# Starlight0798/gymRL

Measured on AMD Instinct MI355X. Metric: env-steps/sec at N envs/GPU (PPO LunarLander), 1/2/4/8 GPUs + %HBM roofline, higher is better.
Workload: dtype f32; 1 GPU; PPO LunarLander-v3, 4096 vectorised envs per MI355X (BASELINE.json configs[1]); envs_per_gpu=4096, rollout_len=2048, num_epochs=10, num_minibatches=32, minibatch=262144, model=ActorCritic 8-256-256-{256-4,256-1} tanh, 200,965 params, parallelism=single GPU

## Files before the change

gymrl_amd/csrc/env_lunar_device.hpp:

```cpp
#pragma once
#include "env_common.hpp"

namespace gymrl {
namespace lunar {


constexpr float kScale = 30.0f;
constexpr float kW = 600.0f / kScale;
constexpr float kH = 400.0f / kScale;
constexpr float kHelipadY = kH / 4.0f;
constexpr float kLegDown = 18.0f / kScale;
constexpr float kLegAway = 20.0f / kScale;
constexpr float kDt = 1.0f / 50.0f;
constexpr int kVelIters = 180, kPosIters = 60, kMaxSteps = 1000;
constexpr float kLinearSlopSqMax = 0x1.a36e30p-16f;
constexpr float kLinearSlop = 0.005f, kAngularSlop = 2.0f / 180.0f * 3.14159265359f;
constexpr float kPolyRadius = 2.0f * kLinearSlop;
constexpr float kMaxLinCorr = 0.2f, kMaxAngCorr = 8.0f / 180.0f * 3.14159265359f;
constexpr float kBaumgarte = 0.2f;
constexpr float kMaxTranslation = 2.0f, kMaxRotation = 0.5f * 3.14159265359f;
constexpr float kTimeToSleep = 0.5f, kLinSleepTol = 0.01f, kAngSleepTol = 2.0f / 180.0f * 3.14159265359f;
constexpr float kMotorTorque = 40.0f;

__device__ constexpr float kInvM[3] = {0.20761245674740486f, 14.0625f, 14.0625f};
// ... 170 lines not shown
    i0x = v1x; i0y = v1y; i1x = v2x; i1y = v2y;
    id0 = 0u | ((uint32_t)pidx << 8) | (0u << 16) | (1u << 24);
    id1 = 0u | ((uint32_t)pidx << 8) | (0u << 16) | (1u << 24);
    ri1 = pidx; ri2 = pidx + 1 < NV ? pidx + 1 : 0;
    rv1x = wx[0]; rv1y = wy[0]; rv2x = wx[0]; rv2y = wy[0]; rnx = wnx[0]; rny = wny[0];
#pragma unroll
    for (int i = 0; i < NV; ++i) {
      if (i == ri1) { rv1x = wx[i]; rv1y = wy[i]; rnx = wnx[i]; rny = wny[i]; }
      if (i == ri2) { rv2x = wx[i]; rv2y = wy[i]; }
    }
  }
  const float sn1x = rny, sn1y = -rnx;
  const float so1 = dot2(sn1x, sn1y, rv1x, rv1y);
  const float so2 = dot2(-sn1x, -sn1y, rv2x, rv2y);

  float c0x, c0y, c1x, c1y; uint32_t cid0, cid1; int np = 0;
  {
    const float d0 = dot2(sn1x, sn1y, i0x, i0y) - so1;
    const float d1 = dot2(sn1x, sn1y, i1x, i1y) - so1;
    c0x = c0y = c1x = c1y = 0.0f; cid0 = cid1 = 0u;
    if (d0 <= 0.0f) { c0x = i0x; c0y = i0y; cid0 = id0; np = 1; }
    if (d1 <= 0.0f) { if (np == 0) { c0x = i1x; c0y = i1y; cid0 = id1; } else { c1x = i1x; c1y = i1y; cid1 = id1; } ++np; }
    if (d0 * d1 < 0.0f) {
      const float t = d0 / (d0 - d1);
      const float nxp = i0x + t * (i1x - i0x), nyp = i0y + t * (i1y - i0y);
      const uint32_t nid = (uint32_t)ri1 | (((id0 >> 8) & 0xFFu) << 8) | (0u << 16) | (1u << 24);
      if (np == 0) { c0x = nxp; c0y = nyp; cid0 = nid; } else { c1x = nxp; c1y = nyp; cid1 = nid; }
      ++np;
    }
  }
  if (np < 2) return;
  float e0x, e0y, e1x, e1y; uint32_t eid0, eid1; np = 0;
  {
    const float d0 = dot2(-sn1x, -sn1y, c0x, c0y) - so2;
    const float d1 = dot2(-sn1x, -sn1y, c1x, c1y) - so2;
    e0x = e0y = e1x = e1y = 0.0f; eid0 = eid1 = 0u;
    if (d0 <= 0.0f) { e0x = c0x; e0y = c0y; eid0 = cid0; np = 1; }
    if (d1 <= 0.0f) { if (np == 0) { e0x = c1x; e0y = c1y; eid0 = cid1; } else { e1x = c1x; e1y = c1y; eid1 = cid1; } ++np; }
    if (d0 * d1 < 0.0f) {
      const float t = d0 / (d0 - d1);
      const float nxp = c0x + t * (c1x - c0x), nyp = c0y + t * (c1y - c0y);
      const uint32_t nid = (uint32_t)ri2 | (((cid0 >> 8) & 0xFFu) << 8) | (0u << 16) | (1u << 24);
      if (np == 0) { e0x = nxp; e0y = nyp; eid0 = nid; } else { e1x = nxp; e1y = nyp; eid1 = nid; }
      ++np;
    }
  }
  if (np < 2) return;

  mf.faceB = use_edge ? 0 : 1;
  if (use_edge) { mf.lnx = rnx; mf.lny = rny; mf.lpx = rv1x; mf.lpy = rv1y; }
  else {
    mf.lnx = NX[0]; mf.lny = NY[0]; mf.lpx = VX[0]; mf.lpy = VY[0];
#pragma unroll
    for (int i = 0; i < NV; ++i) if (i == ri1) { mf.lnx = NX[i]; mf.lny = NY[i]; mf.lpx = VX[i]; mf.lpy = VY[i]; }
  }
  int cnt = 0;
#pragma unroll
  for (int k = 0; k < 2; ++k) {
    const float qx = k == 0 ? e0x : e1x, qy = k == 0 ? e0y : e1y;
    const uint32_t qid = k == 0 ? eid0 : eid1;
    const float sep = dot2(rnx, rny, qx - rv1x, qy - rv1y);
    if (sep <= radius) {
      float lx, ly; uint32_t key;
      if (use_edge) {
        const float dx = qx - px, dy = qy - py;
        lx = qc * dx + qs * dy; ly = -qs * dx + qc * dy;
        key = qid;
      } else {
        lx = qx; ly = qy;
        key = ((qid >> 8) & 0xFFu) | ((qid & 0xFFu) << 8) | (((qid >> 24) & 0xFFu) << 16) | (((qid >> 16) & 0xFFu) << 24);
      }
      if (cnt == 0) { mf.p[0].lpx = lx; mf.p[0].lpy = ly; mf.p[0].key = key; }
      else { mf.p[1].lpx = lx; mf.p[1].lpy = ly; mf.p[1].key = key; }
      ++cnt;
    }
  }
  mf.count = cnt;
}
__device__ __forceinline__ void body_xf(const Body& b, float lcy, float& px, float& py, float& qs, float& qc) {
  det_sincosf(b.a, &qs, &qc);
  px = b.cx - (qc * 0.0f - qs * lcy);
  py = b.cy - (qs * 0.0f + qc * lcy);
}

__device__ __forceinline__ float sel3(int mb, float a, float b, float c) { return mb == 0 ? a : (mb == 1 ? b : c); }
__device__ __forceinline__ Body select_body(const Body (&B)[3], int mb) {
  Body r;
  r.cx = sel3(mb, B[0].cx, B[1].cx, B[2].cx); r.cy = sel3(mb, B[0].cy, B[1].cy, B[2].cy);
  r.a = sel3(mb, B[0].a, B[1].a, B[2].a);
  r.vx = sel3(mb, B[0].vx, B[1].vx, B[2].vx); r.vy = sel3(mb, B[0].vy, B[1].vy, B[2].vy);
  r.w = sel3(mb, B[0].w, B[1].w, B[2].w);
  return r;
}

__device__ __forceinline__ void quad_share_velocity(Body (&B)[3], const Body& mine) {
  B[0].vx = quad_bcast<0>(mine.vx); B[0].vy = quad_bcast<0>(mine.vy); B[0].w = quad_bcast<0>(mine.w);
  B[1].vx = quad_bcast<1>(mine.vx); B[1].vy = quad_bcast<1>(mine.vy); B[1].w = quad_bcast<1>(mine.w);
  B[2].vx = quad_bcast<2>(mine.vx); B[2].vy = quad_bcast<2>(mine.vy); B[2].w = quad_bcast<2>(mine.w);
}
__device__ __forceinline__ void quad_share_position(Body (&B)[3], const Body& mine) {
  B[0].cx = quad_bcast<0>(mine.cx); B[0].cy = quad_bcast<0>(mine.cy); B[0].a = quad_bcast<0>(mine.a);
  B[1].cx = quad_bcast<1>(mine.cx); B[1].cy = quad_bcast<1>(mine.cy); B[1].a = quad_bcast<1>(mine.a);
  B[2].cx = quad_bcast<2>(mine.cx); B[2].cy = quad_bcast<2>(mine.cy); B[2].a = quad_bcast<2>(mine.a);
}

__device__ __forceinline__ void world_step(World& W, const Lds& lds, int role, int action, float disp0,
                                           float disp1, float fx, float fy, float& m_power, float& s_power) {
  Body(&B)[3] = W.b;
  const int mb = role == 3 ? 0 : role;
  const bool is_hull = mb == 0;
  const float mB_ = is_hull ? kInvM[0] : kInvM[1], iB_ = is_hull ? kInvI[0] : kInvI[1];
  const float lcy_ = is_hull ? kHullLcY : 0.0f;
  const float fr_ = is_hull ? sqrtf(0.1f * 0.1f) : sqrtf(0.2f * 0.1f);
  LUNAR_PROF_MARK(pt0);
  m_power = 0.0f; s_power = 0.0f;
  {
    float sn, cs;
    det_sincosf(B[0].a, &sn, &cs);
    const float tipx = sn, tipy = cs, sidex = -cs, sidey = sn;
    const float posx = B[0].cx - (cs * 0.0f - sn * kHullLcY);
    const float posy = B[0].cy - (sn * 0.0f + cs * kHullLcY);
    if (action == 2) {
      m_power = 1.0f;
      const float ox = tipx * (4.0f / kScale + 2.0f * disp0) + sidex * disp1;
      const float oy = -tipy * (4.0f / kScale + 2.0f * disp0) - sidey * disp1;
      const float ipx = posx + ox, ipy = posy + oy;
      const float Ix = -ox * 13.0f * m_power, Iy = -oy * 13.0f * m_power;
      B[0].vx += kInvM[0] * Ix; B[0].vy += kInvM[0] * Iy;
      B[0].w += kInvI[0] * cross2(ipx - B[0].cx, ipy - B[0].cy, Ix, Iy);
    }
    if (action == 1 || action == 3) {
      const float dir = (float)(action - 2);
      s_power = 1.0f;
      const float ox = tipx * disp0 + sidex * (3.0f * disp1 + dir * 12.0f / kScale);
      const float oy = -tipy * disp0 - sidey * (3.0f * disp1 + dir * 12.0f / kScale);
      const float ipx = posx + ox - tipx * 17.0f / kScale;
      const float ipy = posy + oy + tipy * 14.0f / kScale;
      const float Ix = -ox * 0.6f * s_power, Iy = -oy * 0.6f * s_power;
      B[0].vx += kInvM[0] * Ix; B[0].vy += kInvM[0] * Iy;
      B[0].w += kInvI[0] * cross2(ipx - B[0].cx, ipy - B[0].cy, Ix, Iy);
    }
  }

  uint32_t my_touch = 0u;
  bool my_contact = false;
  {
    const Body me = select_body(B, mb);
    float px, py, qs, qc;
    body_xf(me, lcy_, px, py, qs, qc);
    float minx = 3.4e38f, maxx = -3.4e38f, miny = 3.4e38f;
    if (is_hull) {
#pragma unroll
      for (int i = 0; i < 6; ++i) {
        const float x = (qc * kHullVx[i] - qs * kHullVy[i]) + px, y = (qs * kHullVx[i] + qc * kHullVy[i]) + py;
        minx = fminf(minx, x); maxx = fmaxf(maxx, x); miny = fminf(miny, y);
      }
    } else {
#pragma unroll
      for (int i = 0; i < 4; ++i) {
        const float x = (qc * kLegVx[i] - qs * kLegVy[i]) + px, y = (qs * kLegVx[i] + qc * kLegVy[i]) + py;
        minx = fminf(minx, x); maxx = fmaxf(maxx, x); miny = fminf(miny, y);
      }
    }
    int e_lo = (int)floorf((minx - 2.0f * kPolyRadius) * 0.5f);
    int e_hi = (int)floorf((maxx + 2.0f * kPolyRadius) * 0.5f);
    e_lo = e_lo < 0 ? 0 : e_lo;
// ... 241 lines not shown
    P2[L] = lane3(a23, a33, a13); Q2[L] = lane3(a13, a23, a33); A2[L] = lane3(a13, a11, a12);
    P3[L] = lane3(a23, a12, a22); Q3[L] = lane3(a12, a22, a23); A3[L] = lane3(a12, a13, a11);
    A3C[L] = lane3(a13, a23, 0.0f); D2[L] = lane3(a22, a11, 0.0f);
    MBv[L] = lane3(kInvM[L + 1], kInvM[L + 1], kInvI[L + 1]); IBz[L] = r2 ? kInvI[L + 1] : 0.0f;
  }
  const float MAv = lane3(kInvM[0], kInvM[0], kInvI[0]), IAz = r2 ? kInvI[0] : 0.0f;
  float VA = lane3(B[0].vx, B[0].vy, B[0].w);
  float VB[2] = {lane3(B[1].vx, B[1].vy, B[1].w), lane3(B[2].vx, B[2].vy, B[2].w)};
  float JI[2] = {lane3(W.j[0].ix, W.j[0].iy, W.j[0].iz), lane3(W.j[1].ix, W.j[1].iy, W.j[1].iz)};
  float IM[2] = {W.j[0].im, W.j[1].im};
  const float maxImp = h * kMotorTorque;
#define SB __builtin_amdgcn_sched_barrier(0)
#define USEL(c, a, b) (__builtin_unpredictable(c) ? (a) : (b))
  float zb[2];
  zb[1] = quad_perm<0xAA>(JI[1]) * A3C[1];
  zb[0] = 0.0f;
  float lim_nan[2] = {at_limit[0] ? lim_sign[0] : __builtin_nanf(""), at_limit[1] ? lim_sign[1] : __builtin_nanf("")};
  asm volatile("" : "+v"(lim_nan[0]), "+v"(lim_nan[1]));
  auto joints = [&]() {
#pragma unroll
    for (int jj = 0; jj < 2; ++jj) {
      const int L = 1 - jj;
      const bool lim = at_limit[L];
      float t = VB[L] - VA; SB;
      t = t - 0.3f * leg_sign(L); SB;
      float imp = -mmass[L] * t; SB;
      float nw = IM[L] + imp; SB;
      nw = __builtin_amdgcn_fmed3f(nw, -maxImp, maxImp); SB;
      imp = nw - IM[L]; IM[L] = nw; SB;
      const float mb_ = IBz[L] * imp; SB;
      VB[L] = VB[L] + mb_; SB;
      const float ma_ = IAz * imp; SB;
      VA = VA - ma_; SB;
      const float xb = quad_perm<0xAA>(VB[L]) * JPB[L]; SB;
      float c = VB[L] + xb; SB;
      const float xa = quad_perm<0xAA>(VA) * JPA[L]; SB;
      c = c - VA; SB;
      c = c - xa; SB;
      const float u1 = c * C1[L]; SB;
      const float zc = zb[L] - c; SB;
      const float q2 = quad_perm<kRot1>(c) * Q2[L]; SB;
      const float q3 = quad_perm<kRot2>(c) * Q3[L]; SB;
      const float m2 = c * P2[L] - q2; SB;
      const float m3 = c * P3[L] - q3; SB;
      float s1 = quad_perm<kRot1>(u1) + u1; SB;
      const float u2 = A2[L] * m2; SB;
      const float u3 = A3[L] * m3; SB;
      s1 = quad_perm<kRot2>(u1) + s1; SB;
      const float rr = USEL(lim, zc, -c); SB;
      float s2 = quad_perm<kRot1>(u2) + u2; SB;
      float s3 = quad_perm<kRot1>(u3) + u3; SB;
      const float d2r = D2[L] * rr; SB;
      s2 = quad_perm<kRot2>(u2) + s2; SB;
      s3 = quad_perm<kRot2>(u3) + s3; SB;
      const float r2_ = quad_perm<kSwap01>(rr) * K12[L]; SB;
      float sel = USEL(r1, s2, s3); SB;
      sel = USEL(r0, s1, sel); SB;
      const float nsol = -(det3i[L] * sel); SB;
      const float newJ = JI[L] + nsol; SB;
      const float uu = d2r - r2_; SB;
      const float u = det2i[L] * uu; SB;
      const float rt = quad_perm<0xAA>(newJ) * lim_nan[L]; SB;
      const float altz = USEL(lim, -JI[L], 0.0f); SB;
      const float alt = USEL(r2, altz, u); SB;
      float ip;
      asm("v_cmp_nge_f32 vcc, %1, 0\n\tv_cndmask_b32_e32 %0, %2, %3, vcc" : "=v"(ip) : "v"(rt), "v"(nsol), "v"(alt) : "vcc"); SB;
      JI[L] = JI[L] + ip; SB;
      zb[1 - L] = quad_perm<0xAA>(JI[1 - L]) * A3C[1 - L]; SB;
      const float ay = quad_perm<0x55>(ip) * jrAx[L]; SB;
      const float ax = quad_perm<0x00>(ip) * jrAy[L]; SB;
      const float by = quad_perm<0x55>(ip) * jrBx[L]; SB;
      const float bx = quad_perm<0x00>(ip) * jrBy[L]; SB;
      const float crA = ay - ax; SB;
      const float crB = by - bx; SB;
      const float wA = crA + ip; SB;
      const float wB = crB + ip; SB;
      float tA = USEL(r2, wA, ip); SB;
      float tB = USEL(r2, wB, ip); SB;
      tA = MAv * tA; SB;
      tB = MBv[L] * tB; SB;
      VA = VA - tA; SB;
      VB[L] = VB[L] + tB; SB;
    }
  };
#undef SB
#undef USEL
  auto contacts = [&]() {
    if (any_contact) {
      Body me;
      me.cx = me.cy = me.a = 0.0f;
      me.vx = sel3(mb, quad_bcast<0>(VA), quad_bcast<0>(VB[0]), quad_bcast<0>(VB[1]));
      me.vy = sel3(mb, quad_bcast<1>(VA), quad_bcast<1>(VB[0]), quad_bcast<1>(VB[1]));
      me.w = sel3(mb, quad_bcast<2>(VA), quad_bcast<2>(VB[0]), quad_bcast<2>(VB[1]));
#pragma unroll
      for (int s = 0; s < 2; ++s) {
        const int vcount = vcn[s];
        if (vcount > 0) {
          const float nx = vcf[s][VC_NX - 1], ny = vcf[s][VC_NY - 1], tx = ny, ty = -nx;
          const float rx0 = vcf[s][VC_RX0 - 1], ry0 = vcf[s][VC_RY0 - 1], rx1 = vcf[s][VC_RX1 - 1], ry1 = vcf[s][VC_RY1 - 1];
          float ni0 = vim[s][0], ti0 = vim[s][1], ni1 = vim[s][2], ti1 = vim[s][3];
          {
            const float dvx = me.vx + (-me.w * ry0), dvy = me.vy + (me.w * rx0);
            const float vt = dot2(dvx, dvy, tx, ty);
            float lam = vcf[s][VC_TM0 - 1] * (-vt);
            const float maxF = fr_ * ni0;
            const float nw = clampf(ti0 + lam, -maxF, maxF);
            lam = nw - ti0; ti0 = nw;
            const float Px = lam * tx, Py = lam * ty;
            me.vx += mB_ * Px; me.vy += mB_ * Py;
            me.w += iB_ * cross2(rx0, ry0, Px, Py);
          }
          if (vcount == 2) {
            const float dvx = me.vx + (-me.w * ry1), dvy = me.vy + (me.w * rx1);
            const float vt = dot2(dvx, dvy, tx, ty);
            float lam = vcf[s][VC_TM1 - 1] * (-vt);
            const float maxF = fr_ * ni1;
            const float nw = clampf(ti1 + lam, -maxF, maxF);
            lam = nw - ti1; ti1 = nw;
            const float Px = lam * tx, Py = lam * ty;
            me.vx += mB_ * Px; me.vy += mB_ * Py;
            me.w += iB_ * cross2(rx1, ry1, Px, Py);
          }
          if (vcount == 1) {
            const float dvx = me.vx + (-me.w * ry0), dvy = me.vy + (me.w * rx0);
            const float vn = dot2(dvx, dvy, nx, ny);
            float lam = -vcf[s][VC_NM0 - 1] * vn;
            const float nw = fmaxf(ni0 + lam, 0.0f);
            lam = nw - ni0; ni0 = nw;
            const float Px = lam * nx, Py = lam * ny;
            me.vx += mB_ * Px; me.vy += mB_ * Py;
            me.w += iB_ * cross2(rx0, ry0, Px, Py);
          } else {
            const float k11 = vcf[s][VC_K11 - 1], k12 = vcf[s][VC_K12 - 1], k22 = vcf[s][VC_K22 - 1];
            const float a1 = ni0, a2 = ni1;
            const float dv1x = me.vx + (-me.w * ry0), dv1y = me.vy + (me.w * rx0);
            const float dv2x = me.vx + (-me.w * ry1), dv2y = me.vy + (me.w * rx1);
            float vn1 = dot2(dv1x, dv1y, nx, ny), vn2 = dot2(dv2x, dv2y, nx, ny);
            const float b1 = vn1 - (k11 * a1 + k12 * a2);
            const float b2 = vn2 - (k12 * a1 + k22 * a2);
            float x1 = -(vcf[s][VC_I11 - 1] * b1 + vcf[s][VC_I12 - 1] * b2);
            float x2 = -(vcf[s][VC_I12 - 1] * b1 + vcf[s][VC_I22 - 1] * b2);
            bool ok = (x1 >= 0.0f && x2 >= 0.0f);
            if (!ok) {
              x1 = -vcf[s][VC_NM0 - 1] * b1; x2 = 0.0f;
              vn2 = k12 * x1 + b2;
              ok = (x1 >= 0.0f && vn2 >= 0.0f);
            }
            if (!ok) {
              x1 = 0.0f; x2 = -vcf[s][VC_NM1 - 1] * b2;
              vn1 = k12 * x2 + b1;
              ok = (x2 >= 0.0f && vn1 >= 0.0f);
            }
            if (!ok) {
              x1 = 0.0f; x2 = 0.0f;
              ok = (b1 >= 0.0f && b2 >= 0.0f);
            }
            if (ok) {
              const float d1 = x1 - a1, d2 = x2 - a2;
              const float P1x = d1 * nx, P1y = d1 * ny, P2x = d2 * nx, P2y = d2 * ny;
              me.vx += mB_ * (P1x + P2x); me.vy += mB_ * (P1y + P2y);
              me.w += iB_ * (cross2(rx0, ry0, P1x, P1y) + cross2(rx1, ry1, P2x, P2y));
              ni0 = x1; ni1 = x2;
            }
          }
          vim[s][0] = ni0; vim[s][1] = ti0;
          if (vcount == 2) { vim[s][2] = ni1; vim[s][3] = ti1; }
        }
      }
      VA = lane3(quad_bcast<0>(me.vx), quad_bcast<0>(me.vy), quad_bcast<0>(me.w));
      VB[0] = lane3(quad_bcast<1>(me.vx), quad_bcast<1>(me.vy), quad_bcast<1>(me.w));
      VB[1] = lane3(quad_bcast<2>(me.vx), quad_bcast<2>(me.vy), quad_bcast<2>(me.w));
    }
  };
  if (__builtin_amdgcn_ballot_w64(any_contact) == 0ull) {
#pragma nounroll
    for (int it = 0; it < kVelIters; ++it) joints();
  } else {
#pragma nounroll
    for (int it = 0; it < kVelIters; ++it) { joints(); contacts(); }
  }
  B[0].vx = quad_bcast<0>(VA); B[0].vy = quad_bcast<1>(VA); B[0].w = quad_bcast<2>(VA);
#pragma unroll
  for (int L = 0; L < 2; ++L) {
    B[L + 1].vx = quad_bcast<0>(VB[L]); B[L + 1].vy = quad_bcast<1>(VB[L]); B[L + 1].w = quad_bcast<2>(VB[L]);
    W.j[L].ix = quad_bcast<0>(JI[L]); W.j[L].iy = quad_bcast<1>(JI[L]); W.j[L].iz = quad_bcast<2>(JI[L]);
    W.j[L].im = quad_bcast<2>(IM[L]);
  }
  LUNAR_PROF_MARK(pt3);
  LUNAR_PROF_ADD(lds, 2, pt2, pt3);
#ifdef GYMRL_LUNAR_PROF
  const bool wave_contact = __builtin_amdgcn_ballot_w64(any_contact) != 0ull;
  LUNAR_PROF_ADD(lds, wave_contact ? 6 : 7, pt2, pt3);
#endif
  if (my_contact) {
#pragma unroll
    for (int s = 0; s < 2; ++s) {
      if (vcn[s] > 0) {
        lds.mf(s, MF_P0 + P_NI) = vim[s][0]; lds.mf(s, MF_P0 + P_TI) = vim[s][1];
        if (vcn[s] == 2) { lds.mf(s, MF_P1 + P_NI) = vim[s][2]; lds.mf(s, MF_P1 + P_TI) = vim[s][3]; }
      }
    }
  }

#pragma unroll
  for (int b = 0; b < 3; ++b) {
    float tx = h * B[b].vx, ty = h * B[b].vy;
    if (dot2(tx, ty, tx, ty) > kMaxTranslation * kMaxTranslation) {
      const float ratio = kMaxTranslation / sqrtf(dot2(tx, ty, tx, ty));
      B[b].vx *= ratio; B[b].vy *= ratio;
    }
    const float rot = h * B[b].w;
    if (rot * rot > kMaxRotation * kMaxRotation) {
      const float ratio = kMaxRotation / fabsf(rot);
      B[b].w *= ratio;
    }
    B[b].cx += h * B[b].vx; B[b].cy += h * B[b].vy; B[b].a += h * B[b].w;
  }

  LUNAR_PROF_MARK(pt4);
  LUNAR_PROF_ADD(lds, 3, pt3, pt4);
#ifdef GYMRL_LUNAR_PROF
  int prof_pos_iters = 0;
#endif
  bool position_solved = false;
  float plim_value[2], plim_slop[2], plim_lo[2], plim_hi[2];
#pragma unroll
  for (int L = 0; L < 2; ++L) {
    const bool lower = W.j[L].state == 1;
    plim_value[L] = lower ? joint_lower(L) : joint_upper(L);
    plim_slop[L] = lower ? kAngularSlop : -kAngularSlop;
    plim_lo[L] = lower ? -kMaxAngCorr : 0.0f;
    plim_hi[L] = lower ? 0.0f : kMaxAngCorr;
  }
  int pcnt[2] = {0, 0};
  bool pfaceB[2] = {false, false};
  float plnx[2], plny[2], plpx[2], plpy[2], pqx[2][2], pqy[2][2];
#pragma unroll
  for (int s = 0; s < 2; ++s) {
    plnx[s] = plny[s] = plpx[s] = plpy[s] = 0.0f;
    pqx[s][0] = pqx[s][1] = pqy[s][0] = pqy[s][1] = 0.0f;
    if (my_contact) {
      pcnt[s] = (int)lds.mu(s, MF_COUNT);
      pfaceB[s] = lds.mu(s, MF_FACEB) != 0u;
      plnx[s] = lds.mf(s, MF_LNX); plny[s] = lds.mf(s, MF_LNY);
      plpx[s] = lds.mf(s, MF_LPX); plpy[s] = lds.mf(s, MF_LPY);
#pragma unroll
      for (int k = 0; k < 2; ++k) {
        pqx[s][k] = lds.mf(s, MF_P0 + 5 * k + P_LPX); pqy[s][k] = lds.mf(s, MF_P0 + 5 * k + P_LPY);
      }
    }
  }
#pragma nounroll
  for (int it = 0; it < kPosIters; ++it) {
    float min_sep = 0.0f;
    if (any_contact) {
      Body me = select_body(B, mb);
      float my_min = 0.0f;
#pragma unroll
      for (int s = 0; s < 2; ++s) {
        const int cnt = pcnt[s];
        if (cnt > 0) {
          const bool faceB = pfaceB[s];
          const float lnx = plnx[s], lny = plny[s], lpx = plpx[s], lpy = plpy[s];
#pragma unroll
          for (int k = 0; k < 2; ++k) {
            if (k < cnt) {
              const float qx = pqx[s][k], qy = pqy[s][k];
              float px, py, qs, qc;
              body_xf(me, lcy_, px, py, qs, qc);
              float nx, ny, ptx, pty, sep;
              if (!faceB) {
                nx = lnx; ny = lny;
                const float clx = (qc * qx - qs * qy) + px, cly = (qs * qx + qc * qy) + py;
                sep = dot2(clx - lpx, cly - lpy, nx, ny) - kPolyRadius - kPolyRadius;
                ptx = clx; pty = cly;
// ... 414 lines not shown
```

gymrl_amd/csrc/rollout_lunar.hip:

```cpp
#include "env_lunar_device.hpp"
#include "mlp_device.hpp"
#include "policy_device.hpp"
#include "mhc_policy_device.hpp"

using namespace gymrl;
using namespace gymrl::lunar;
namespace M = gymrl::mlp;

namespace {

constexpr int kThreads = M::kWaves * 64;
constexpr int kActions = 4, kObs = 8;
constexpr int kGaeChunk = 16;
constexpr int kDynFloats = M::kBufs * M::kRows * M::kStride + M::kRows * M::kInStride + M::kRows * M::kHeadStride;
constexpr int kDynBytes = 96 * 1024;
constexpr int kDynBytesMhc = 32 * 1024;
static_assert(kDynFloats * 4 <= kDynBytes, "LDS carve-up");

__global__ __launch_bounds__(kThreads) void rollout_lunar_kernel(gymrl_rollout_lunar_args a, gymrl_mlp_desc d) {
  extern __shared__ __attribute__((aligned(16))) float dyn_lds[];
  __shared__ uint32_t lds_words[kLdsWords * kEnvBlock];
  __shared__ uint32_t lds_words_refill[kLdsWords * kEnvBlock];
  __shared__ uint32_t lds_park[kParkWords * kEnvBlock];
  float (*lds)[M::kRows * M::kStride] = reinterpret_cast<float (*)[M::kRows * M::kStride]>(dyn_lds);
  float* xin = dyn_lds + M::kBufs * M::kRows * M::kStride;
  float* head = xin + M::kRows * M::kInStride;
  const int tid = threadIdx.x, wave = tid >> 6, lane = tid & 63;
  const int N = a.n_envs, T = a.T;
  const int m0 = blockIdx.x * M::kRows;
  const int t_end = a.t0 + a.nsteps;
  const int role = lane & 3, row = lane >> 2, i = m0 + row;
  const bool valid = i < N;
  const LunarState st(a.env_state, N);
#ifdef GYMRL_LUNAR_PROF
  constexpr int kProfSlots = 24;
  unsigned long long* const wprof = a.wg_ticks ? reinterpret_cast<unsigned long long*>(a.wg_ticks) + 2 * gridDim.x + kProfSlots * blockIdx.x : nullptr;
  Lds slds_{lds_words + lane, wprof, lds_park + lane};
  if (a.wg_ticks && valid) { slds_.envp = reinterpret_cast<unsigned long long*>(a.wg_ticks) + (2 + kProfSlots) * gridDim.x + i; slds_.envn = N; }
  const Lds slds = slds_;
  if (wprof && lane == 0) {
    wprof[20 + wave] = (unsigned long long)__builtin_amdgcn_s_getreg(4 | (31 << 11)) |
                       ((unsigned long long)__builtin_amdgcn_s_getreg(20 | (31 << 11)) << 32);
  }
#else
  const Lds slds{lds_words + lane, lds_park + lane};
#endif
#ifdef GYMRL_LUNAR_PROF
  const Lds rlds{lds_words_refill + lane, nullptr};
#else
  const Lds rlds{lds_words_refill + lane};
#endif
  const double gl = (double)(float)(a.gamma * a.lam);
  if (a.wg_ticks && tid == 0) a.wg_ticks[2 * blockIdx.x] = wall_clock64();

  for (int e = tid; e < M::kRows * M::kInStride; e += kThreads) xin[e] = 0.0f;
  __syncthreads();
  for (int e = tid; e < M::kRows * kObs; e += kThreads) {
    const int r = e / kObs, c = e - r * kObs;
    if (m0 + r < N) xin[r * M::kInStride + c] = a.obs[((size_t)a.t0 * N + m0 + r) * kObs + c];
  }
  const uint32_t vdefer = M::deferrable_stages(d, kActions);
  for (int t = a.t0; t <= t_end; ++t) {
    const bool tail = t == t_end;
    if (tail && t_end != T) break;
    LUNAR_PROF_MARK(rtb);
    __syncthreads();
    LUNAR_PROF_MARK(rt0);
    if (wave == 0) LUNAR_PROF_ADD(slds, 16, rtb, rt0);
    M::forward_tile(d, lds, xin, head, m0, N, tid, vdefer);
    LUNAR_PROF_MARK(rt1);
    if (wave == 0) LUNAR_PROF_ADD(slds, 8, rt0, rt1);
    auto value_part = [&]() {
      const float v = head[row * M::kHeadStride + kActions];
      if (valid && role == 0) {
        if (a.gae_running && t > 0) {
          const int tp = t - 1;
          const size_t o = (size_t)tp * N + i;
          double2* agg = reinterpret_cast<double2*>(a.gae_workspace) + (size_t)(tp / kGaeChunk) * N;
          gae_online_compose(a.rew[o], a.done[o], a.val[o], v, a.gamma, gl, (tp % kGaeChunk) == 0,
                             (tp % kGaeChunk) == kGaeChunk - 1 || tp == T - 1, a.gae_running, agg, N, i);
        }
        if (tail) {
          a.next_value[i] = v;
          if (a.gae_carry && a.gae_running) {
            const int C = (T + kGaeChunk - 1) / kGaeChunk;
            const double2* agg0 = reinterpret_cast<const double2*>(a.gae_workspace);
            static_assert(sizeof(lds_words_refill) >= sizeof(double2) * kGaeCarrySeg * kEnvBlock / 4, "carry scratch");
            gae_carry_scan(agg0, C, N, i, reinterpret_cast<double*>(const_cast<double2*>(agg0) + (size_t)C * N),
                           reinterpret_cast<double2*>(lds_words_refill) + row, kEnvBlock / 4);
          }
        } else a.val[(size_t)t * N + i] = v;
      }
    };
    if (wave == 2 && vdefer) {
      M::forward_deferred(d, lds, head, m0, N, lane, vdefer);
      value_part();
#ifdef GYMRL_LUNAR_PROF
      if (wprof && lane == 0) wprof[17] += wall_clock64() - rt1;
#endif
    }
    const bool refill_wave = wave == 1;
    if (wave == 0 || (refill_wave && !tail && a.refill)) {
      int act = 0;
      if (!refill_wave) {
        float z[kActions];
#pragma unroll
        for (int k = 0; k < kActions; ++k) z[k] = head[row * M::kHeadStride + k];
        if (!vdefer) value_part();
        if (!tail) {
          float lp, H;
          const size_t o = (size_t)t * N + (valid ? i : 0);
          act = categorical_pick<kActions>(z, a.noise_exp ? a.noise_exp + o * kActions : nullptr, a.seed,
                                           (uint64_t)(a.env_id0 + i), a.counter0 + (uint64_t)t, 0, lp, H);
          if (valid && role == 0) { a.act[o] = act; a.logp[o] = lp; }
        }
      }
      if (!tail) {
        const StepOut out{a.obs + (size_t)(t + 1) * N * kObs, nullptr, a.rew + (size_t)t * N, nullptr, nullptr,
// ... 190 lines not shown
```

Measured before the change: 7.092 million env-steps/s.

## Add specialized resting-contact velocity solver path for single-point leg contacts

Adds a specialized velocity-iteration path for waves where every contacting lane is a leg with exactly one contact point. It replaces the general contacts() lambda with a compact one-point friction+normal solve done directly on quad-distributed velocities, skipping the broadcast and reassembly of the general path. It also adds profiling counters and enlarges the profile slot count under the profiling macro. The risk is a numerical mismatch against the general solver, plus extra register pressure from the precomputed resting-contact values.

```diff
diff --git a/gymrl_amd/csrc/env_lunar_device.hpp b/gymrl_amd/csrc/env_lunar_device.hpp
--- a/gymrl_amd/csrc/env_lunar_device.hpp
+++ b/gymrl_amd/csrc/env_lunar_device.hpp
@@ -683,6 +683,83 @@
       VA = VA - tA; SB;
       VB[L] = VB[L] + tB; SB;
     }
+  };
+  const bool rs_slot1 = vcn[0] == 0;
+  auto rs_vc = [&](int f) { return rs_slot1 ? vcf[1][f - 1] : vcf[0][f - 1]; };
+  const float rs_nx = rs_vc(VC_NX), rs_ny = rs_vc(VC_NY), rs_tx = rs_ny, rs_ty = -rs_nx;
+  const float rs_rx = rs_vc(VC_RX0), rs_ry = rs_vc(VC_RY0), rs_tm = rs_vc(VC_TM0), rs_nm = rs_vc(VC_NM0);
+  const float rs_mB = kInvM[1], rs_iB = kInvI[1], rs_fr = sqrtf(0.2f * 0.1f);
+  float rs_ni = rs_slot1 ? vim[1][0] : vim[0][0], rs_ti = rs_slot1 ? vim[1][1] : vim[0][1];
+  const bool rs_has0 = quad_bcast_u<1>(my_contact ? 1u : 0u) != 0u, rs_has1 = quad_bcast_u<2>(my_contact ? 1u : 0u) != 0u;
+  const bool rs_0x = rs_has0 && r0, rs_0y = rs_has0 && r1, rs_0w = rs_has0 && r2;
+  const bool rs_1x = rs_has1 && r0, rs_1y = rs_has1 && r1, rs_1w = rs_has1 && r2;
+  auto resting = [&]() {
+    const float in_x1 = quad_bcast<0>(VB[1]); SB;
+    const float in_y1 = quad_bcast<1>(VB[1]); SB;
+    const float in_w0 = quad_bcast<2>(VB[0]); SB;
+    const float in_x0 = quad_bcast<0>(VB[0]); SB;
+    float vy = USEL(r1, VB[0], in_y1); SB;
+    float w = USEL(r2, VB[1], in_w0); SB;
+    float vx = USEL(r1, in_x0, in_x1); SB;
+    {
+      const float wy = -w * rs_ry; SB;
+      const float wx = w * rs_rx; SB;
+      const float dvx = vx + wy; SB;
+      const float dvy = vy + wx; SB;
+      const float p1 = dvx * rs_tx; SB;
+      const float p2 = dvy * rs_ty; SB;
+      const float vt = p1 + p2; SB;
+      float lam = rs_tm * (-vt); SB;
+      const float maxF = rs_fr * rs_ni; SB;
+      const float su = rs_ti + lam; SB;
+      const float nw = clampf(su, -maxF, maxF); SB;
+      lam = nw - rs_ti; rs_ti = nw; SB;
+      const float Px = lam * rs_tx; SB;
+      const float Py = lam * rs_ty; SB;
+      const float ax = rs_mB * Px; SB;
+      const float ay = rs_mB * Py; SB;
+      vx = vx + ax; SB;
+      vy = vy + ay; SB;
+      const float c1 = rs_rx * Py; SB;
+      const float c2 = rs_ry * Px; SB;
+      const float cr = c1 - c2; SB;
+      const float aw = rs_iB * cr; SB;
+      w = w + aw; SB;
+    }
+    {
+      const float wy = -w * rs_ry; SB;
+      const float wx = w * rs_rx; SB;
+      const float dvx = vx + wy; SB;
+      const float dvy = vy + wx; SB;
+      const float p1 = dvx * rs_nx; SB;
+      const float p2 = dvy * rs_ny; SB;
+      const float vn = p1 + p2; SB;
+      float lam = -rs_nm * vn; SB;
+      const float su = rs_ni + lam; SB;
+      const float nw = fmaxf(su, 0.0f); SB;
+      lam = nw - rs_ni; rs_ni = nw; SB;
+      const float Px = lam * rs_nx; SB;
+      const float Py = lam * rs_ny; SB;
+      const float ax = rs_mB * Px; SB;
+      const float ay = rs_mB * Py; SB;
+      vx = vx + ax; SB;
+      vy = vy + ay; SB;
+      const float c1 = rs_rx * Py; SB;
+      const float c2 = rs_ry * Px; SB;
+      const float cr = c1 - c2; SB;
+      const float aw = rs_iB * cr; SB;
+      w = w + aw; SB;
+    }
+    const float out_x0 = quad_bcast<1>(vx); SB;
+    const float out_x1 = quad_bcast<2>(vx); SB;
+    const float out_y1 = quad_bcast<2>(vy); SB;
+    const float out_w0 = quad_bcast<1>(w); SB;
+    VB[0] = USEL(rs_0y, vy, VB[0]); SB;
+    VB[1] = USEL(rs_1w, w, VB[1]); SB;
+    VB[0] = USEL(rs_0x, out_x0, VB[0]); SB;
+    VB[1] = USEL(rs_1x, out_x1, VB[1]); SB;
+    VB[1] = USEL(rs_1y, out_y1, VB[1]); SB;
+    VB[0] = USEL(rs_0w, out_w0, VB[0]); SB;
   };
 #undef SB
 #undef USEL
@@ -773,9 +850,15 @@
       VB[1] = lane3(quad_bcast<2>(me.vx), quad_bcast<2>(me.vy), quad_bcast<2>(me.w));
     }
   };
+  const bool lane_general = my_contact && (is_hull || vcn[0] + vcn[1] != 1);
+  const bool wave_resting = __builtin_amdgcn_ballot_w64(my_contact) != 0ull && __builtin_amdgcn_ballot_w64(lane_general) == 0ull;
   if (__builtin_amdgcn_ballot_w64(any_contact) == 0ull) {
 #pragma nounroll
     for (int it = 0; it < kVelIters; ++it) joints();
+  } else if (wave_resting) {
+#pragma nounroll
+    for (int it = 0; it < kVelIters; ++it) { joints(); resting(); }
+    if (rs_slot1) { vim[1][0] = rs_ni; vim[1][1] = rs_ti; } else { vim[0][0] = rs_ni; vim[0][1] = rs_ti; }
   } else {
 #pragma nounroll
     for (int it = 0; it < kVelIters; ++it) { joints(); contacts(); }
@@ -792,6 +875,21 @@
 #ifdef GYMRL_LUNAR_PROF
   const bool wave_contact = __builtin_amdgcn_ballot_w64(any_contact) != 0ull;
   LUNAR_PROF_ADD(lds, wave_contact ? 6 : 7, pt2, pt3);
+  if (lds.prof && (threadIdx.x & 63) == 0) {
+    lds.prof[24] += wave_resting ? 1ull : 0ull; lds.prof[25] += (wave_contact && !wave_resting) ? 1ull : 0ull;
+    lds.prof[26] += wave_resting ? pt3 - pt2 : 0ull;
+  }
+  {
+    const bool one_mf = my_contact && !is_hull && (vcn[0] == 0 || vcn[1] == 0);
+    const bool one_pt = one_mf && vcn[0] + vcn[1] == 1, two_pt = one_mf && vcn[0] + vcn[1] == 2;
+    const unsigned long long mc = __builtin_amdgcn_ballot_w64(my_contact && role != 3), m1 = __builtin_amdgcn_ballot_w64(one_mf),
+                             mp = __builtin_amdgcn_ballot_w64(one_pt), m2 = __builtin_amdgcn_ballot_w64(two_pt);
+    if (lds.prof && (threadIdx.x & 63) == 0) {
+      lds.prof[27] += (mc != 0ull && m2 == mc) ? 1ull : 0ull; lds.prof[28] += (mc != 0ull && m1 == mc && mp != mc && m2 != mc) ? 1ull : 0ull;
+      lds.prof[29] += (unsigned long long)__builtin_popcountll(mc); lds.prof[30] += (unsigned long long)__builtin_popcountll(mp);
+      lds.prof[31] += (unsigned long long)__builtin_popcountll(m2);
+    }
+  }
 #endif
   if (my_contact) {
 #pragma unroll
diff --git a/gymrl_amd/csrc/rollout_lunar.hip b/gymrl_amd/csrc/rollout_lunar.hip
--- a/gymrl_amd/csrc/rollout_lunar.hip
+++ b/gymrl_amd/csrc/rollout_lunar.hip
@@ -33,7 +33,7 @@
   const bool valid = i < N;
   const LunarState st(a.env_state, N);
 #ifdef GYMRL_LUNAR_PROF
-  constexpr int kProfSlots = 24;
+  constexpr int kProfSlots = 32;
   unsigned long long* const wprof = a.wg_ticks ? reinterpret_cast<unsigned long long*>(a.wg_ticks) + 2 * gridDim.x + kProfSlots * blockIdx.x : nullptr;
   Lds slds_{lds_words + lane, wprof, lds_park + lane};
   if (a.wg_ticks && valid) { slds_.envp = reinterpret_cast<unsigned long long*>(a.wg_ticks) + (2 + kProfSlots) * gridDim.x + i; slds_.envn = N; }
```

New measurement: 7.278 million env-steps/s, median of 6. 1.03x the previous value.

## Specialize contact solver per wave contact pattern with branchless selects

Applied to the files above, without the earlier changes.

The velocity-iteration contact solver becomes a template specialised on slot count, one- versus two-point manifolds and hull contact. Wave-wide ballots pick the cheapest variant for the whole 180-iteration loop. Inside each variant the data-dependent branches (point count, the block-solver LCP cases) are replaced by computing every candidate and choosing with unpredictable selects, which removes divergence. The cost is redundant arithmetic per lane and more code size and register pressure, and the reordered block-solver cases could subtly change results if the selection logic is wrong.

```diff
diff --git a/gymrl_amd/csrc/env_lunar_device.hpp b/gymrl_amd/csrc/env_lunar_device.hpp
--- a/gymrl_amd/csrc/env_lunar_device.hpp
+++ b/gymrl_amd/csrc/env_lunar_device.hpp
@@ -276,6 +276,8 @@
   px = b.cx - (qc * 0.0f - qs * lcy);
   py = b.cy - (qs * 0.0f + qc * lcy);
 }
+
+template <int V> struct IntC { static constexpr int value = V; };
 
 __device__ __forceinline__ float sel3(int mb, float a, float b, float c) { return mb == 0 ? a : (mb == 1 ? b : c); }
 __device__ __forceinline__ Body select_body(const Body (&B)[3], int mb) {
@@ -686,99 +688,124 @@
   };
 #undef SB
 #undef USEL
-  auto contacts = [&]() {
-    if (any_contact) {
-      Body me;
-      me.cx = me.cy = me.a = 0.0f;
-      me.vx = sel3(mb, quad_bcast<0>(VA), quad_bcast<0>(VB[0]), quad_bcast<0>(VB[1]));
-      me.vy = sel3(mb, quad_bcast<1>(VA), quad_bcast<1>(VB[0]), quad_bcast<1>(VB[1]));
-      me.w = sel3(mb, quad_bcast<2>(VA), quad_bcast<2>(VB[0]), quad_bcast<2>(VB[1]));
-#pragma unroll
-      for (int s = 0; s < 2; ++s) {
-        const int vcount = vcn[s];
-        if (vcount > 0) {
-          const float nx = vcf[s][VC_NX - 1], ny = vcf[s][VC_NY - 1], tx = ny, ty = -nx;
-          const float rx0 = vcf[s][VC_RX0 - 1], ry0 = vcf[s][VC_RY0 - 1], rx1 = vcf[s][VC_RX1 - 1], ry1 = vcf[s][VC_RY1 - 1];
-          float ni0 = vim[s][0], ti0 = vim[s][1], ni1 = vim[s][2], ti1 = vim[s][3];
-          {
-            const float dvx = me.vx + (-me.w * ry0), dvy = me.vy + (me.w * rx0);
-            const float vt = dot2(dvx, dvy, tx, ty);
-            float lam = vcf[s][VC_TM0 - 1] * (-vt);
-            const float maxF = fr_ * ni0;
-            const float nw = clampf(ti0 + lam, -maxF, maxF);
-            lam = nw - ti0; ti0 = nw;
-            const float Px = lam * tx, Py = lam * ty;
-            me.vx += mB_ * Px; me.vy += mB_ * Py;
-            me.w += iB_ * cross2(rx0, ry0, Px, Py);
-          }
-          if (vcount == 2) {
-            const float dvx = me.vx + (-me.w * ry1), dvy = me.vy + (me.w * rx1);
-            const float vt = dot2(dvx, dvy, tx, ty);
-            float lam = vcf[s][VC_TM1 - 1] * (-vt);
-            const float maxF = fr_ * ni1;
-            const float nw = clampf(ti1 + lam, -maxF, maxF);
-            lam = nw - ti1; ti1 = nw;
-            const float Px = lam * tx, Py = lam * ty;
-            me.vx += mB_ * Px; me.vy += mB_ * Py;
-            me.w += iB_ * cross2(rx1, ry1, Px, Py);
-          }
-          if (vcount == 1) {
-            const float dvx = me.vx + (-me.w * ry0), dvy = me.vy + (me.w * rx0);
-            const float vn = dot2(dvx, dvy, nx, ny);
-            float lam = -vcf[s][VC_NM0 - 1] * vn;
-            const float nw = fmaxf(ni0 + lam, 0.0f);
-            lam = nw - ni0; ni0 = nw;
-            const float Px = lam * nx, Py = lam * ny;
-            me.vx += mB_ * Px; me.vy += mB_ * Py;
-            me.w += iB_ * cross2(rx0, ry0, Px, Py);
-          } else {
-            const float k11 = vcf[s][VC_K11 - 1], k12 = vcf[s][VC_K12 - 1], k22 = vcf[s][VC_K22 - 1];
-            const float a1 = ni0, a2 = ni1;
-            const float dv1x = me.vx + (-me.w * ry0), dv1y = me.vy + (me.w * rx0);
-            const float dv2x = me.vx + (-me.w * ry1), dv2y = me.vy + (me.w * rx1);
-            float vn1 = dot2(dv1x, dv1y, nx, ny), vn2 = dot2(dv2x, dv2y, nx, ny);
-            const float b1 = vn1 - (k11 * a1 + k12 * a2);
-            const float b2 = vn2 - (k12 * a1 + k22 * a2);
-            float x1 = -(vcf[s][VC_I11 - 1] * b1 + vcf[s][VC_I12 - 1] * b2);
-            float x2 = -(vcf[s][VC_I12 - 1] * b1 + vcf[s][VC_I22 - 1] * b2);
-            bool ok = (x1 >= 0.0f && x2 >= 0.0f);
-            if (!ok) {
-              x1 = -vcf[s][VC_NM0 - 1] * b1; x2 = 0.0f;
-              vn2 = k12 * x1 + b2;
-              ok = (x1 >= 0.0f && vn2 >= 0.0f);
-            }
-            if (!ok) {
-              x1 = 0.0f; x2 = -vcf[s][VC_NM1 - 1] * b2;
-              vn1 = k12 * x2 + b1;
-              ok = (x2 >= 0.0f && vn1 >= 0.0f);
-            }
-            if (!ok) {
-              x1 = 0.0f; x2 = 0.0f;
-              ok = (b1 >= 0.0f && b2 >= 0.0f);
-            }
-            if (ok) {
-              const float d1 = x1 - a1, d2 = x2 - a2;
-              const float P1x = d1 * nx, P1y = d1 * ny, P2x = d2 * nx, P2y = d2 * ny;
-              me.vx += mB_ * (P1x + P2x); me.vy += mB_ * (P1y + P2y);
-              me.w += iB_ * (cross2(rx0, ry0, P1x, P1y) + cross2(rx1, ry1, P2x, P2y));
-              ni0 = x1; ni1 = x2;
-            }
-          }
-          vim[s][0] = ni0; vim[s][1] = ti0;
-          if (vcount == 2) { vim[s][2] = ni1; vim[s][3] = ti1; }
+  bool c_use[2], c_two[2], c_one[2];
+#pragma unroll
+  for (int s = 0; s < 2; ++s) { c_use[s] = vcn[s] > 0; c_two[s] = vcn[s] == 2; c_one[s] = vcn[s] == 1; }
+#define USEL(c, a, b) (__builtin_unpredictable(c) ? (a) : (b))
+  auto contacts = [&](auto slots_c, auto one_c, auto two_c, auto hull_c) {
+    constexpr int kSlots = decltype(slots_c)::value;
+    constexpr bool kOne = decltype(one_c)::value, kTwo = decltype(two_c)::value, kHull = decltype(hull_c)::value;
+    static_assert(kOne || kTwo, "a manifold has one point or two");
+    float vx, vy, w;
+    if constexpr (kHull) {
+      vx = sel3(mb, quad_bcast<0>(VA), quad_bcast<0>(VB[0]), quad_bcast<0>(VB[1]));
+      vy = sel3(mb, quad_bcast<1>(VA), quad_bcast<1>(VB[0]), quad_bcast<1>(VB[1]));
+      w = sel3(mb, quad_bcast<2>(VA), quad_bcast<2>(VB[0]), quad_bcast<2>(VB[1]));
+    } else {
+      const float x0 = quad_bcast<0>(VB[0]), x1 = quad_bcast<0>(VB[1]), y0 = quad_bcast<1>(VB[0]), y1 = quad_bcast<1>(VB[1]);
+      const float z0 = quad_bcast<2>(VB[0]), z1 = quad_bcast<2>(VB[1]);
+      vx = USEL(r1, x0, x1); vy = USEL(r1, y0, y1); w = USEL(r1, z0, z1);
+    }
+#pragma unroll
+    for (int s = 0; s < kSlots; ++s) {
+      const float nx = vcf[s][VC_NX - 1], ny = vcf[s][VC_NY - 1], tx = ny, ty = -nx;
+      const float rx0 = vcf[s][VC_RX0 - 1], ry0 = vcf[s][VC_RY0 - 1], rx1 = vcf[s][VC_RX1 - 1], ry1 = vcf[s][VC_RY1 - 1];
+      float ni0 = vim[s][0], ti0 = vim[s][1], ni1 = vim[s][2], ti1 = vim[s][3];
+      float cvx = vx, cvy = vy, cw = w;
+      {
+        const float dvx = cvx + (-cw * ry0), dvy = cvy + (cw * rx0);
+        const float vt = dot2(dvx, dvy, tx, ty);
+        float lam = vcf[s][VC_TM0 - 1] * (-vt);
+        const float maxF = fr_ * ni0;
+        const float nw = clampf(ti0 + lam, -maxF, maxF);
+        lam = nw - ti0; ti0 = nw;
+        const float Px = lam * tx, Py = lam * ty;
+        cvx += mB_ * Px; cvy += mB_ * Py;
+        cw += iB_ * cross2(rx0, ry0, Px, Py);
+      }
+      if constexpr (kTwo) {
+        const float dvx = cvx + (-cw * ry1), dvy = cvy + (cw * rx1);
+        const float vt = dot2(dvx, dvy, tx, ty);
+        float lam = vcf[s][VC_TM1 - 1] * (-vt);
+        const float maxF = fr_ * ni1;
+        const float nw = clampf(ti1 + lam, -maxF, maxF);
+        lam = nw - ti1; ti1 = nw;
+        const float Px = lam * tx, Py = lam * ty;
+        const float fvx = cvx + mB_ * Px, fvy = cvy + mB_ * Py;
+        const float fw = cw + iB_ * cross2(rx1, ry1, Px, Py);
+        if constexpr (kOne) { cvx = USEL(c_two[s], fvx, cvx); cvy = USEL(c_two[s], fvy, cvy); cw = USEL(c_two[s], fw, cw); }
+        else { cvx = fvx; cvy = fvy; cw = fw; }
+      }
+      const float dv1x = cvx + (-cw * ry0), dv1y = cvy + (cw * rx0);
+      float vn1 = dot2(dv1x, dv1y, nx, ny);
+      float ovx = cvx, ovy = cvy, ow = cw, oni = ni0;
+      if constexpr (kOne) {
+        float lam = -vcf[s][VC_NM0 - 1] * vn1;
+        const float nw = fmaxf(ni0 + lam, 0.0f);
+        lam = nw - ni0; oni = nw;
+        const float Px = lam * nx, Py = lam * ny;
+        ovx = cvx + mB_ * Px; ovy = cvy + mB_ * Py;
+        ow = cw + iB_ * cross2(rx0, ry0, Px, Py);
+      }
+      if constexpr (kTwo) {
+        const float k11 = vcf[s][VC_K11 - 1], k12 = vcf[s][VC_K12 - 1], k22 = vcf[s][VC_K22 - 1];
+        const float a1 = ni0, a2 = ni1;
+        const float dv2x = cvx + (-cw * ry1), dv2y = cvy + (cw * rx1);
+        const float vn2 = dot2(dv2x, dv2y, nx, ny);
+        const float b1 = vn1 - (k11 * a1 + k12 * a2);
+        const float b2 = vn2 - (k12 * a1 + k22 * a2);
+        const float xm1 = -(vcf[s][VC_I11 - 1] * b1 + vcf[s][VC_I12 - 1] * b2);
+        const float xm2 = -(vcf[s][VC_I12 - 1] * b1 + vcf[s][VC_I22 - 1] * b2);
+        const float xa1 = -vcf[s][VC_NM0 - 1] * b1, va2 = k12 * xa1 + b2;
+        const float xb2 = -vcf[s][VC_NM1 - 1] * b2, vb1 = k12 * xb2 + b1;
+        const bool okm = xm1 >= 0.0f && xm2 >= 0.0f;
+        const bool oka = xa1 >= 0.0f && va2 >= 0.0f;
+        const bool okb = xb2 >= 0.0f && vb1 >= 0.0f;
+        const bool okc = b1 >= 0.0f && b2 >= 0.0f;
+        const bool ok = okm || oka || okb || okc;
+        const float x1 = USEL(okm, xm1, USEL(oka, xa1, 0.0f));
+        const float x2 = USEL(okm, xm2, USEL(oka, 0.0f, USEL(okb, xb2, 0.0f)));
+        const float d1 = x1 - a1, d2 = x2 - a2;
+        const float P1x = d1 * nx, P1y = d1 * ny, P2x = d2 * nx, P2y = d2 * ny;
+        const float bvx = cvx + mB_ * (P1x + P2x), bvy = cvy + mB_ * (P1y + P2y);
+        const float bw = cw + iB_ * (cross2(rx0, ry0, P1x, P1y) + cross2(rx1, ry1, P2x, P2y));
+        if constexpr (kOne) {
+          const bool blk = c_two[s] && ok;
+          const bool one = c_one[s];
+          cvx = USEL(blk, bvx, USEL(one, ovx, cvx)); cvy = USEL(blk, bvy, USEL(one, ovy, cvy)); cw = USEL(blk, bw, USEL(one, ow, cw));
+          ni0 = USEL(blk, x1, USEL(c_one[s], oni, ni0)); ni1 = USEL(blk, x2, ni1);
+        } else {
+          cvx = USEL(ok, bvx, cvx); cvy = USEL(ok, bvy, cvy); cw = USEL(ok, bw, cw);
+          ni0 = USEL(ok, x1, ni0); ni1 = USEL(ok, x2, ni1);
         }
-      }
-      VA = lane3(quad_bcast<0>(me.vx), quad_bcast<0>(me.vy), quad_bcast<0>(me.w));
-      VB[0] = lane3(quad_bcast<1>(me.vx), quad_bcast<1>(me.vy), quad_bcast<1>(me.w));
-      VB[1] = lane3(quad_bcast<2>(me.vx), quad_bcast<2>(me.vy), quad_bcast<2>(me.w));
-    }
+      } else {
+        cvx = ovx; cvy = ovy; cw = ow; ni0 = oni;
+      }
+      vim[s][0] = ni0; vim[s][1] = ti0; vim[s][2] = ni1; vim[s][3] = ti1;
+      vx = USEL(c_use[s], cvx, vx); vy = USEL(c_use[s], cvy, vy); w = USEL(c_use[s], cw, w);
+    }
+    auto lane2 = [&](float x, float y, float z) { return r0 ? x : (r1 ? y : z); };
+    if constexpr (kHull) VA = lane2(quad_bcast<0>(vx), quad_bcast<0>(vy), quad_bcast<0>(w));
+    VB[0] = lane2(quad_bcast<1>(vx), quad_bcast<1>(vy), quad_bcast<1>(w));
+    VB[1] = lane2(quad_bcast<2>(vx), quad_bcast<2>(vy), quad_bcast<2>(w));
   };
-  if (__builtin_amdgcn_ballot_w64(any_contact) == 0ull) {
+#undef USEL
+  const unsigned long long w_any = __builtin_amdgcn_ballot_w64(any_contact);
+  const unsigned long long w_slot1 = __builtin_amdgcn_ballot_w64(c_use[1]);
+  const unsigned long long w_two = __builtin_amdgcn_ballot_w64(c_two[0] || c_two[1]);
+  const unsigned long long w_hull = __builtin_amdgcn_ballot_w64(is_hull && my_contact);
+  if (w_any == 0ull) {
 #pragma nounroll
     for (int it = 0; it < kVelIters; ++it) joints();
+  } else if ((w_slot1 | w_hull | w_two) == 0ull) {
+#pragma nounroll
+    for (int it = 0; it < kVelIters; ++it) { joints(); contacts(IntC<1>{}, IntC<1>{}, IntC<0>{}, IntC<0>{}); }
+  } else if ((w_slot1 | w_hull) == 0ull) {
+#pragma nounroll
+    for (int it = 0; it < kVelIters; ++it) { joints(); contacts(IntC<1>{}, IntC<1>{}, IntC<1>{}, IntC<0>{}); }
   } else {
 #pragma nounroll
-    for (int it = 0; it < kVelIters; ++it) { joints(); contacts(); }
+    for (int it = 0; it < kVelIters; ++it) { joints(); contacts(IntC<2>{}, IntC<1>{}, IntC<1>{}, IntC<1>{}); }
   }
   B[0].vx = quad_bcast<0>(VA); B[0].vy = quad_bcast<1>(VA); B[0].w = quad_bcast<2>(VA);
 #pragma unroll
```

New measurement: 7.153 million env-steps/s before, 7.005 million env-steps/s after. 2.1% lower.
